# shayneobrien/generative-models

Measured on NVIDIA H100. Metric: train_step_images_per_sec, higher is better.
Workload: dtype bf16

## Files before the change

### generative-models_b200/gm_b200/csrc/engine.cu

```cuda
#include <cstdarg>
#include <cstdio>
#include <cstring>
#include <map>
#include <string>
#include <vector>

#include "gm_b200.h"
#include "gemm_wgmma.cuh"
#include "kernels.cuh"
#include "conv_ops.cuh"

using namespace gm;

typedef CUresult (*PFN_encodeTiled)(CUtensorMap*, CUtensorMapDataType, cuuint32_t, void*, const cuuint64_t*,
                                    const cuuint64_t*, const cuuint32_t*, const cuuint32_t*, CUtensorMapInterleave,
                                    CUtensorMapSwizzle, CUtensorMapL2promotion, CUtensorMapFloatOOBfill);

struct gm_ctx {
  int device = 0;
  int num_sms = 0;
  PFN_encodeTiled encode = nullptr;
  std::string err;
  long long launches = 0;
  float* scratch = nullptr;
// ... 22 lines not shown
    if (e__ != cudaSuccess)                                                                       \
      return fail(ctx, GM_ERR_CUDA, "%s failed: %s (%s:%d)", #expr, cudaGetErrorString(e__), __FILE__, __LINE__); \
  } while (0)

static inline int cdiv(int a, int b) { return (a + b - 1) / b; }
static inline int rup(int a, int b) { return cdiv(a, b) * b; }

static inline uint64_t splitmix64(uint64_t x) {
  x += 0x9E3779B97F4A7C15ull; x = (x ^ (x >> 30)) * 0xBF58476D1CE4E5B9ull; x = (x ^ (x >> 27)) * 0x94D049BB133111EBull;
  return x ^ (x >> 31);
}
static Sampler make_sampler(long long n, uint64_t seed, uint64_t round, uint64_t offset, const unsigned long long* step_ptr = nullptr) {
  Sampler sp;
  sp.n = n > 0 ? unsigned(n) : 0u;
  int bits = 2;
  while (bits < 32 && (1ull << bits) < (unsigned long long)(n > 0 ? n : 1)) ++bits;
  if (bits & 1) ++bits;
  sp.half_bits = unsigned(bits / 2);
  sp.seed_mix = splitmix64(seed);
  sp.key = sampler_key(sp.seed_mix, round);
  sp.offset = offset;
  sp.step_ptr = step_ptr;
  return sp;
}
static const Sampler kNoSampler = {0u, 1u, 0ull, 0ull, nullptr, 0ull};

static int make_tmap(gm_ctx* c, CUtensorMap* tm, const void* ptr, uint64_t inner, uint64_t outer, uint64_t ld,
                     uint32_t box_inner, uint32_t box_outer, CUtensorMapSwizzle swizzle = CU_TENSOR_MAP_SWIZZLE_128B) {
  if ((reinterpret_cast<uintptr_t>(ptr) & 15) || (ld * 2) % 16 != 0)
    return fail(c, GM_ERR_ARG, "tensor map: pointer/ld must be 16-byte aligned (ptr=%p ld=%llu)", ptr, (unsigned long long)ld);
  cuuint64_t dims[2] = {inner, outer};
  cuuint64_t strides[1] = {ld * 2};
  cuuint32_t box[2] = {box_inner, box_outer};
  cuuint32_t estr[2] = {1, 1};
  CUresult r = c->encode(tm, CU_TENSOR_MAP_DATA_TYPE_BFLOAT16, 2, const_cast<void*>(ptr), dims, strides, box, estr,
                         CU_TENSOR_MAP_INTERLEAVE_NONE, swizzle, CU_TENSOR_MAP_L2_PROMOTION_L2_256B,
                         CU_TENSOR_MAP_FLOAT_OOB_FILL_NONE);
  if (r != CUDA_SUCCESS) return fail(c, GM_ERR_CUDA, "cuTensorMapEncodeTiled failed with %d", int(r));
  return GM_OK;
}

enum PlanKind { PK_NT_208 = 0, PK_NT_64, PK_TN_256, PK_TN_64 };

struct GemmPlan {
  CUtensorMap tmA, tmB;
  CUtensorMap tmA2, tmB2;
  mutable CUtensorMap tmC;
  mutable int tmc_state;
  GemmParams p;
  int kind;
  int grid;
  double flops;
};

static bool g_pdl = true;
static bool g_tma_store = true;
struct ProfAll { const char* name; cudaEvent_t e0, e1; };
static bool g_prof_all = false;
static std::vector<ProfAll> g_prof_all_recs;
template <typename... KArgs, typename... Args>
static cudaError_t launch_pdl(const char* name, void (*kern)(KArgs...), dim3 grid, dim3 block, size_t smem, cudaStream_t s, Args&&... args) {
  struct Scope {
    cudaStream_t s; ProfAll r; bool on;
    Scope(const char* n, cudaStream_t s_) : s(s_), on(g_prof_all) {
      if (on) { r.name = n; cudaEventCreate(&r.e0); cudaEventCreate(&r.e1); cudaEventRecord(r.e0, s); }
    }
    ~Scope() { if (on) { cudaEventRecord(r.e1, s); g_prof_all_recs.push_back(r); } }
  } scope(name, s);
  const bool pdl = g_pdl && strcmp(name, "xhat_kernel") != 0;
  cudaLaunchConfig_t cfg;
  memset(&cfg, 0, sizeof cfg);
  cfg.gridDim = grid;
  cfg.blockDim = block;
  cfg.dynamicSmemBytes = smem;
  cfg.stream = s;
  cudaLaunchAttribute at[1];
  at[0].id = cudaLaunchAttributeProgrammaticStreamSerialization;
  at[0].val.programmaticStreamSerializationAllowed = 1;
  cfg.attrs = at;
  cfg.numAttrs = pdl ? 1 : 0;
  return cudaLaunchKernelEx(&cfg, kern, KArgs(args)...);
}

template <int BN, bool AMN, bool BMN, int ACT_T = -1, int AUX_T = -1, int BIAS_T = -1, int DOT_T = -1, bool SPLIT = false>
static cudaError_t launch_inst(const GemmPlan& pl, cudaStream_t s) {
  using Cfg = GemmCfg<BN, !AMN>;
  constexpr int CL = kGemmCluster<BN, AMN, BMN>;
  auto kern = gemm_wgmma_kernel<BN, AMN, BMN, ACT_T, AUX_T, BIAS_T, DOT_T, SPLIT>;
  cudaLaunchConfig_t cfg;
  memset(&cfg, 0, sizeof cfg);
  cfg.gridDim = dim3(pl.grid);
  cfg.blockDim = dim3(kGemmThreads);
  cfg.dynamicSmemBytes = Cfg::SMEM_BYTES;
  cfg.stream = s;
  cudaLaunchAttribute at[2];
  int na = 0;
  if (CL > 1) {
    at[na].id = cudaLaunchAttributeClusterDimension;
    at[na].val.clusterDim.x = CL;
    at[na].val.clusterDim.y = 1;
    at[na].val.clusterDim.z = 1;
    ++na;
  }
  static bool configured[64] = {};
  static int max_clusters[64] = {};
  int dev = 0;
  cudaGetDevice(&dev);
  const bool cached = dev >= 0 && dev < 64;
  int mc = cached ? max_clusters[dev] : 0;
  if (!cached || !configured[dev]) {
    cudaError_t e = cudaFuncSetAttribute(kern, cudaFuncAttributeMaxDynamicSharedMemorySize, Cfg::SMEM_BYTES);
    if (e != cudaSuccess) return e;
    if (CL > 1) {
      cfg.gridDim = dim3(CL);
      cfg.attrs = at;
      cfg.numAttrs = na;
      e = cudaOccupancyMaxActiveClusters(&mc, kern, &cfg);
      if (e != cudaSuccess) return e;
      if (mc < 1) return cudaErrorInvalidConfiguration;
    }
    if (cached) { max_clusters[dev] = mc; configured[dev] = true; }
  }
  if (CL > 1) {
    const GemmParams& q = pl.p;
    const int items = cdiv(q.m_tiles, CL) * q.n_tiles * q.splits;
    cfg.gridDim = dim3(CL * (items < mc ? items : mc));
  }
  if (g_pdl) {
    at[na].id = cudaLaunchAttributeProgrammaticStreamSerialization;
    at[na].val.programmaticStreamSerializationAllowed = 1;
    ++na;
  }
  cfg.attrs = at;
  cfg.numAttrs = na;
  GemmParams prm = pl.p;
  prm.tma_store = pl.tmc_state == 1 ? 1 : 0;
  prm.f32_vec = prm.epi == EPI_F32 && !(reinterpret_cast<uintptr_t>(prm.part) & 15) && prm.ldp % 4 == 0 && prm.part_stride % 4 == 0;
  return cudaLaunchKernelEx(&cfg, kern, pl.tmA, pl.tmB, pl.tmC, pl.tmA2, pl.tmB2, prm);
}

template <int BN, bool AMN, bool BMN>
static cudaError_t launch_split(const GemmPlan& pl, cudaStream_t s) {
  return launch_inst<BN, AMN, BMN, -1, -1, -1, -1, true>(pl, s);
}

static cudaError_t launch_nt208(const GemmPlan& pl, cudaStream_t s) {
  const GemmParams& p = pl.p;
  const bool bias = p.bias != nullptr, dot = p.dot_w != nullptr;
  const int aux = p.aux_mode;
  if (p.epi != EPI_BF16) return launch_inst<208, false, false>(pl, s);
  if (p.dot_sq && (bias || dot || aux != AUX_NONE || p.act != ACT_NONE)) return launch_inst<208, false, false>(pl, s);
  if (bias && !dot && aux == AUX_NONE && p.act == ACT_RELU) return launch_inst<208, false, false, ACT_RELU, AUX_NONE, 1, 0>(pl, s);
  if (bias && !dot && aux == AUX_NONE && p.act == ACT_SIGMOID) return launch_inst<208, false, false, ACT_SIGMOID, AUX_NONE, 1, 0>(pl, s);
  if (bias && dot && p.dot_mask == 1 && aux == AUX_NONE && p.act == ACT_RELU) return launch_inst<208, false, false, ACT_RELU, AUX_NONE, 1, 3>(pl, s);
  if (bias && dot && p.dot_mask == 3 && aux == AUX_NONE && p.act == ACT_RELU) return launch_inst<208, false, false, ACT_RELU, AUX_NONE, 1, 5>(pl, s);
  if (p.dot_mask) return launch_inst<208, false, false>(pl, s);
  if (bias && dot && aux == AUX_NONE && p.act == ACT_RELU) return launch_inst<208, false, false, ACT_RELU, AUX_NONE, 1, 1>(pl, s);
  if (!bias && !dot && aux == AUX_SIGMOID_GRAD && p.act == ACT_NONE) return launch_inst<208, false, false, ACT_NONE, AUX_SIGMOID_GRAD, 0, 0>(pl, s);
  if (!bias && !dot && aux == AUX_RELU_MASK && p.act == ACT_NONE) return launch_inst<208, false, false, ACT_NONE, AUX_RELU_MASK, 0, 0>(pl, s);
  if (!bias && !dot && aux == AUX_NONZERO_MASK && p.act == ACT_NONE) return launch_inst<208, false, false, ACT_NONE, AUX_NONZERO_MASK, 0, 0>(pl, s);
  if (bias && !dot && aux == AUX_L1 && p.act == ACT_NONE) return launch_inst<208, false, false, ACT_NONE, AUX_L1, 1, 0>(pl, s);
  if (bias && !dot && aux == AUX_VAE_OUT && p.act == ACT_SIGMOID) return launch_inst<208, false, false, ACT_SIGMOID, AUX_VAE_OUT, 1, 0>(pl, s);
  if (!bias && !dot && aux == AUX_NONE && p.act == ACT_NONE && p.dot_sq) return launch_inst<208, false, false, ACT_NONE, AUX_NONE, 0, 2>(pl, s);
  if (!bias && !dot && aux == AUX_NONE && p.act == ACT_NONE) return launch_inst<208, false, false, ACT_NONE, AUX_NONE, 0, 0>(pl, s);
  return launch_inst<208, false, false>(pl, s);
}

static int launch_plan(gm_ctx* c, const GemmPlan& pl, cudaStream_t s) {
  if (pl.tmc_state == 0) {
    const GemmParams& p = pl.p;
    const bool nt = pl.kind == PK_NT_208 || pl.kind == PK_NT_64;
    pl.tmc_state = 2;
    const bool plain = p.aux_mode == AUX_NONE && p.dot_w == nullptr && p.dot_sq == 0;
    if (g_tma_store && nt && plain && p.nparts == 1 && p.epi == EPI_BF16 && p.out != nullptr && !(reinterpret_cast<uintptr_t>(p.out) & 15) &&
        (p.ldo * 2) % 16 == 0 && p.out_cols > 0) {
      int rc = make_tmap(c, &pl.tmC, p.out, uint64_t(p.out_cols), uint64_t(p.M), uint64_t(p.ldo), kEpiCols, kEpiRows, CU_TENSOR_MAP_SWIZZLE_64B);
      if (rc) return rc;
      pl.tmc_state = 1;
    }
  }
  cudaError_t e;
  gm_ctx::ProfRec rec;
  ProfAll pa;
  if (g_prof_all) {
    static const char* kKind[4] = {"gemm_nt208", "gemm_nt64", "gemm_tn256", "gemm_tn64"};
    static std::map<int, std::string> names;
    const GemmParams& q = pl.p;
    const int key = pl.kind | (q.act << 4) | (q.aux_mode << 8) | ((q.dot_w != nullptr) << 12) | (q.dot_sq << 14) |
                    ((q.bias != nullptr) << 15) | ((q.epi == EPI_F32) << 16) | ((q.K >= 512) << 17) | ((q.nparts == 3) << 18) | (q.dot_mask << 19);
    auto it = names.find(key);
    if (it == names.end()) {
      char buf[128];
      snprintf(buf, sizeof buf, "%s[act%d aux%d%s%s%s%s%s K%s%s]", kKind[pl.kind], q.act, q.aux_mode, q.bias ? " bias" : "", q.dot_w ? " dot" : "",
               q.dot_mask == 3 ? " pre" : (q.dot_mask ? " mask" : ""), q.dot_sq ? " sq" : "", q.epi == EPI_F32 ? " f32" : "", q.K >= 512 ? "long" : "short", q.nparts == 3 ? " split" : "");
      it = names.emplace(key, buf).first;
    }
    pa.name = it->second.c_str();
    cudaEventCreate(&pa.e0); cudaEventCreate(&pa.e1);
    cudaEventRecord(pa.e0, s);
  }
  if (c->prof) {
    cudaEventCreate(&rec.e0);
    cudaEventCreate(&rec.e1);
    rec.kind = pl.kind;
    rec.flops = pl.flops;
    cudaEventRecord(rec.e0, s);
  }
  if (pl.p.nparts == 3) {
    switch (pl.kind) {
      case PK_NT_208: e = launch_split<208, false, false>(pl, s); break;
      case PK_NT_64: e = launch_split<64, false, false>(pl, s); break;
      case PK_TN_256: e = launch_split<256, true, true>(pl, s); break;
      default: e = launch_split<64, true, true>(pl, s); break;
    }
  } else
  switch (pl.kind) {
    case PK_NT_208: e = launch_nt208(pl, s); break;
    case PK_NT_64: e = launch_inst<64, false, false>(pl, s); break;
    case PK_TN_256: e = launch_inst<256, true, true>(pl, s); break;
    default: e = launch_inst<64, true, true>(pl, s); break;
  }
  c->launches++;
  if (c->prof) {
    cudaEventRecord(rec.e1, s);
    c->prof_recs.push_back(rec);
  }
  if (g_prof_all) { cudaEventRecord(pa.e1, s); g_prof_all_recs.push_back(pa); }
  if (e != cudaSuccess) return fail(c, GM_ERR_CUDA, "GEMM launch failed: %s", cudaGetErrorString(e));
  return GM_OK;
}

static int plan_gemm(gm_ctx* c, GemmPlan* pl, int mode, int M, int N, int K, const void* A, int lda, const void* B,
                     int ldb, int ncover, int max_splits) {
  memset(pl, 0, sizeof *pl);
  if (M <= 0 || N <= 0 || K <= 0) return fail(c, GM_ERR_ARG, "gemm: bad extents %d %d %d", M, N, K);
  int bn, boxn = 0;
  if (mode == 0) {
    if (ncover <= 64) { pl->kind = PK_NT_64; bn = 64; boxn = 64; }
    else { pl->kind = PK_NT_208; bn = 208; boxn = 208 / kGemmCluster<208, false, false>; }
    int rc = make_tmap(c, &pl->tmA, A, K, M, lda, BK, BM);
    if (rc) return rc;
    rc = make_tmap(c, &pl->tmB, B, K, N, ldb, BK, boxn);
    if (rc) return rc;
  } else {
    if (ncover <= 64) { pl->kind = PK_TN_64; bn = 64; }
    else { pl->kind = PK_TN_256; bn = 256; }
    int rc = make_tmap(c, &pl->tmA, A, M, K, lda, 64, BK);
    if (rc) return rc;
    rc = make_tmap(c, &pl->tmB, B, N, K, ldb, 64, BK);
    if (rc) return rc;
  }
  GemmParams& p = pl->p;
  pl->flops = 2.0 * M * N * K;
  p.M = M; p.N = N; p.K = K;
  p.m_tiles = cdiv(M, BM);
  p.n_tiles = cdiv(ncover, bn);
  p.kblocks = cdiv(K, BK);
  p.nparts = 1; p.kb_part = p.kblocks; p.lo_off = 0;
  pl->tmA2 = pl->tmA; pl->tmB2 = pl->tmB;
  if (c->plan_lo > 0) {
    const __nv_bfloat16* A2 = static_cast<const __nv_bfloat16*>(A) + c->plan_lo;
    const __nv_bfloat16* B2 = static_cast<const __nv_bfloat16*>(B) + c->plan_lo;
    int rc;
    if (mode == 0) {
      if ((rc = make_tmap(c, &pl->tmA2, A2, K, M, lda, BK, BM))) return rc;
      if ((rc = make_tmap(c, &pl->tmB2, B2, K, N, ldb, BK, boxn))) return rc;
    } else {
      if ((rc = make_tmap(c, &pl->tmA2, A2, M, K, lda, 64, BK))) return rc;
      if ((rc = make_tmap(c, &pl->tmB2, B2, N, K, ldb, 64, BK))) return rc;
    }
    p.nparts = 3; p.kblocks = 3 * p.kb_part; p.lo_off = c->plan_lo;
  }
  const int tiles = p.m_tiles * p.n_tiles;
  const int slots = c->num_sms;
  int splits = 1;
  if (max_splits > 1) {
    splits = slots / tiles;
    if (splits > max_splits) splits = max_splits;
    if (splits > p.kblocks) splits = p.kblocks;
    if (splits < 1) splits = 1;
  }
  p.kb_per_split = cdiv(p.kblocks, splits);
  p.splits = cdiv(p.kblocks, p.kb_per_split);
  const int total = tiles * p.splits;
  pl->grid = total < slots ? total : slots;
  return GM_OK;
}

__global__ void reduce_partials_kernel(const float* __restrict__ part, int nsplit, long long stride, long long rows, int cols,
                                       int ld, float* __restrict__ out) {
  griddep_sync();
  const long long k = blockIdx.x * (long long)blockDim.x + threadIdx.x;
  if (k >= rows * cols) return;
  const long long i = cols == ld ? k : (k / cols) * ld + k % cols;
  float t = 0.f;
  for (int s0 = 0; s0 < nsplit; s0 += 8) {
    float a[8];
#pragma unroll
    for (int u = 0; u < 8; ++u) a[u] = (s0 + u < nsplit) ? part[i + (long long)(s0 + u) * stride] : 0.f;
#pragma unroll
    for (int u = 0; u < 8; ++u) t += a[u];
  }
  out[i] = t;
}

extern "C" int gm_version(void) { return 100; }

extern "C" int gm_ctx_create(int device, gm_ctx** out) {
  if (!out) return GM_ERR_ARG;
  *out = nullptr;
  gm_ctx* c = new gm_ctx();
  c->device = device;
  *out = c;
  int n = 0;
  if (cudaGetDeviceCount(&n) != cudaSuccess || n <= 0)
    return fail(c, GM_ERR_CUDA, "no CUDA device visible: this library has no CPU fallback");
  CU_OK(c, cudaSetDevice(device));
  cudaDeviceProp prop;
  CU_OK(c, cudaGetDeviceProperties(&prop, device));
  if (prop.major != 9 || prop.minor != 0)
    return fail(c, GM_ERR_UNSUPPORTED, "device is sm_%d%d; this library is built for sm_90a (H100) only", prop.major, prop.minor);
  c->num_sms = prop.multiProcessorCount;
  void* fn = nullptr;
  cudaDriverEntryPointQueryResult q;
  CU_OK(c, cudaGetDriverEntryPoint("cuTensorMapEncodeTiled", &fn, cudaEnableDefault, &q));
  if (!fn || q != cudaDriverEntryPointSuccess) return fail(c, GM_ERR_CUDA, "cuTensorMapEncodeTiled not available");
  c->encode = reinterpret_cast<PFN_encodeTiled>(fn);
  const char* np = getenv("GM_NO_PDL");
  g_pdl = !(np && np[0] == '1');
  const char* nts = getenv("GM_NO_TMA_STORE");
  g_tma_store = !(nts && nts[0] == '1');
  return GM_OK;
}
extern "C" int gm_ctx_destroy(gm_ctx* c) {
  if (!c) return GM_OK;
  if (c->scratch) cudaFree(c->scratch);
  if (c->red) cudaFree(c->red);
  if (c->loss_zero) cudaFree(c->loss_zero);
  delete c;
  return GM_OK;
}
extern "C" const char* gm_last_error(const gm_ctx* c) { return c ? c->err.c_str() : "null ctx"; }
extern "C" int gm_ctx_num_sms(const gm_ctx* c) { return c ? c->num_sms : 0; }
extern "C" long long gm_launch_count(gm_ctx* c, int reset) {
  if (!c) return 0;
  const long long n = c->launches;
  if (reset) c->launches = 0;
  return n;
// ... 1219 lines not shown
```

### generative-models_b200/gm_b200/csrc/gemm_wgmma.cuh

```cuda
#pragma once
#include "ptx.cuh"

namespace gm {

constexpr int BM = 128;
constexpr int BK = 64;
constexpr int kMmaK = 16;
constexpr int kProducerThreads = 128;
constexpr int kConsumerWarps = 8;
constexpr int kGemmThreads = kProducerThreads + kConsumerWarps * 32;
constexpr int kProducerRegs = 40;
constexpr int kConsumerRegs = 232;
static_assert(kProducerThreads * kProducerRegs + kConsumerWarps * 32 * kConsumerRegs <= 65536, "register file");
constexpr int kSmemBudget = 227 * 1024;

enum : int { EPI_BF16 = 0, EPI_F32 = 1 };
enum : int { ACT_NONE = 0, ACT_RELU = 1, ACT_SIGMOID = 2, ACT_LRELU = 3 };
enum : int { AUX_NONE = 0, AUX_SIGMOID_GRAD = 1, AUX_RELU_MASK = 2, AUX_VAE_OUT = 3, AUX_L1 = 4, AUX_NONZERO_MASK = 5 };

struct GemmParams {
  int M, N, K;
  int m_tiles, n_tiles;
  int splits, kblocks, kb_per_split;
  int epi;
  __nv_bfloat16* out;
  int ldo;
  int out_cols;
  int pad_one;
  const float* bias;
  int act;
  const __nv_bfloat16* aux;
  int ld_aux;
  int aux_mode;
  const float* dot_w;
  int dot_sq;
  const float* row_scale;
  int row_split;
  int dot_mask;
  int tma_store;
  const float* row_vec;
  float* dot_out;
  int dot_ld;
  float* part;
  long long part_stride;
  int ldp;
  int transpose;
  int f32_vec;
  int nparts, kb_part;
  long long lo_off;
  float act_slope;
};

constexpr int kEpiRows = 16;
constexpr int kEpiStep = 64;
constexpr int kEpiCols = 32;
constexpr int kEpiScratchBytes = kEpiRows * kEpiStep * 4;
constexpr int kEpiPitch = 144;
constexpr int kEpiVecBlocks = 8;
constexpr int kEpiVecBytes = kEpiVecBlocks * kEpiCols * 4 * 2;
static_assert(kEpiRows * kEpiPitch <= kEpiScratchBytes && 2 * kEpiRows * kEpiCols * 2 <= kEpiScratchBytes, "staging");
__device__ __forceinline__ uint32_t frag_swz(int r) { return uint32_t(((r & 3) << 1) | ((r >> 2) & 1)); }

template <int BN_, bool STAGED_EPI = true>
struct GemmCfg {
  static constexpr int BN = BN_;
  static constexpr int A_BYTES = BM * BK * 2;
  static constexpr int B_BYTES = BN * BK * 2;
  static constexpr int STAGE_BYTES = A_BYTES + B_BYTES;
  static constexpr int EPI_BYTES = kConsumerWarps * (kEpiScratchBytes + (STAGED_EPI ? kEpiVecBytes : 0));
  static_assert(!STAGED_EPI || (BN + kEpiCols - 1) / kEpiCols <= kEpiVecBlocks, "bias/dot staging too small");
  static constexpr int FIXED_BYTES = 1024 + 512 + EPI_BYTES;
  static constexpr int STAGES_RAW = (kSmemBudget - FIXED_BYTES) / STAGE_BYTES;
  static constexpr int STAGES = STAGES_RAW > 8 ? 8 : STAGES_RAW;
  static constexpr int SMEM_BYTES = STAGES * STAGE_BYTES + FIXED_BYTES;
  static constexpr int BOXN = BN;
  static_assert(BN % 16 == 0 && BN <= 256, "wgmma N constraint (and 16-column epilogue chunks)");
  static_assert(STAGES >= 2, "need a pipeline");
  static_assert(BN < 208 || STAGES >= 4, "the 208- and 256-wide kernels need a 4-stage ring to hide TMA latency");
};

template <int BN, bool A_MN, bool B_MN>
constexpr int kGemmCluster = (BN == 208 && !A_MN && !B_MN) ? 2 : 1;

template <int BN, bool A_MN, bool B_MN, int ACT_T = -1, int AUX_T = -1, int BIAS_T = -1, int DOT_T = -1, bool SPLIT = false>
__global__ void __launch_bounds__(kGemmThreads, 1)
gemm_wgmma_kernel(const __grid_constant__ CUtensorMap tmA, const __grid_constant__ CUtensorMap tmB,
                  const __grid_constant__ CUtensorMap tmC, const __grid_constant__ CUtensorMap tmA2,
                  const __grid_constant__ CUtensorMap tmB2, const GemmParams p) {
  static_assert(!SPLIT || ACT_T < 0, "split operands: universal epilogue only");
  using Cfg = GemmCfg<BN, !A_MN>;
  constexpr int STAGES = Cfg::STAGES;
  constexpr int CL = kGemmCluster<BN, A_MN, B_MN>;
  static_assert(!B_MN || BN % 64 == 0, "MN-major B needs 64-wide atoms");
  static_assert(CL == 1 || (!B_MN && (BN / CL) % 8 == 0 && (Cfg::B_BYTES / CL) % 1024 == 0), "multicast B share");

  extern __shared__ uint8_t smem_raw[];
  const uint32_t smem_base = (smem_u32(smem_raw) + 1023u) & ~1023u;
  const uint32_t bar_base = smem_base + STAGES * Cfg::STAGE_BYTES;
  auto full_bar = [&](int s) { return bar_base + 8u * s; };
  auto empty_bar = [&](int s) { return bar_base + 8u * (STAGES + s); };
  const uint32_t epi_base = bar_base + 512u;

  const int warp = __shfl_sync(0xffffffffu, int(threadIdx.x >> 5), 0);
  const int lane = threadIdx.x & 31;

  griddep_launch();
  if (warp == 0 && lane == 0) {
    tma_prefetch_desc(&tmA);
    tma_prefetch_desc(&tmB);
    if constexpr (SPLIT) { tma_prefetch_desc(&tmA2); tma_prefetch_desc(&tmB2); }
    if (p.tma_store) tma_prefetch_desc(&tmC);
    for (int s = 0; s < STAGES; ++s) {
      mbar_init(full_bar(s), 1);
      mbar_init(empty_bar(s), CL * kConsumerWarps);
    }
    fence_mbar_init();
  }
  if constexpr (CL > 1) cluster_sync();
  else __syncthreads();
  griddep_wait();

  const int rank = CL > 1 ? int(cluster_ctarank()) : 0;
  const int tiles = (p.m_tiles + CL - 1) / CL * p.n_tiles;
  const int total = tiles * p.splits;
  const int first = blockIdx.x / CL, stride = gridDim.x / CL;

  if (warp < kProducerThreads / 32) {
    setmaxnreg_dec<kProducerRegs>();
    if (warp == 0) {
      int stage = 0;
      uint32_t phase = 0;
      const bool leader = elect_one();
      for (int item = first; item < total; item += stride) {
        const int split = item / tiles;
        const int rem = item - split * tiles;
        const int m0 = ((rem / p.n_tiles) * CL + rank) * BM;
        const int n0 = (rem % p.n_tiles) * BN;
        const int kb0 = split * p.kb_per_split;
        const int kb1 = min(kb0 + p.kb_per_split, p.kblocks);
        for (int kb = kb0; kb < kb1; ++kb) {
          mbar_wait(empty_bar(stage), phase ^ 1u);
          if (leader) {
            const uint32_t a_dst = smem_base + stage * Cfg::STAGE_BYTES;
            const uint32_t b_dst = a_dst + Cfg::A_BYTES;
            int kk = kb, opart = 0;
            if constexpr (SPLIT) { opart = kb / p.kb_part; kk = kb - opart * p.kb_part; }
            const CUtensorMap* const ta = (SPLIT && opart == 2) ? &tmA2 : &tmA;
            const CUtensorMap* const tb = (SPLIT && opart == 1) ? &tmB2 : &tmB;
            const int k0 = kk * BK;
            mbar_arrive_expect_tx(full_bar(stage), Cfg::STAGE_BYTES);
            if constexpr (!A_MN) {
              tma_load_2d(a_dst, ta, full_bar(stage), k0, m0);
            } else {
#pragma unroll
              for (int a = 0; a < BM / 64; ++a)
                tma_load_2d(a_dst + a * (BK * 128), ta, full_bar(stage), m0 + a * 64, k0);
            }
            if constexpr (CL > 1) {
              tma_load_2d_multicast(b_dst + rank * (Cfg::B_BYTES / CL), tb, full_bar(stage), k0, n0 + rank * (BN / CL), (1u << CL) - 1);
            } else if constexpr (!B_MN) {
              tma_load_2d(b_dst, tb, full_bar(stage), k0, n0);
            } else {
#pragma unroll
              for (int b = 0; b < BN / 64; ++b)
                tma_load_2d(b_dst + b * (BK * 128), tb, full_bar(stage), n0 + b * 64, k0);
            }
          }
          __syncwarp();
          if (++stage == STAGES) { stage = 0; phase ^= 1u; }
        }
      }
    }
  } else {
    setmaxnreg_inc<kConsumerRegs>();
    const int cw = warp - kProducerThreads / 32;
    const int wg = cw >> 2;
    const int er = lane & 15;
    const int par = lane >> 4;
    const uint32_t scratch_s = epi_base + uint32_t(cw) * kEpiScratchBytes;
    const uint32_t vec_s = epi_base + kConsumerWarps * kEpiScratchBytes + uint32_t(cw) * kEpiVecBytes;
    const int act = ACT_T >= 0 ? ACT_T : p.act;
    const int aux_mode = AUX_T >= 0 ? AUX_T : p.aux_mode;
    const bool has_bias = BIAS_T >= 0 ? (BIAS_T != 0) : (p.bias != nullptr);
    const bool has_dot = DOT_T >= 0 ? (DOT_T == 1 || DOT_T == 3 || DOT_T == 5) : (p.dot_w != nullptr);
    const bool store_pre = DOT_T >= 0 ? (DOT_T == 5) : (p.dot_mask == 3);
    const bool mask_all = DOT_T >= 0 ? (DOT_T == 3) : (p.dot_mask == 1);
    const bool has_sq = DOT_T >= 0 ? (DOT_T == 2) : (p.dot_sq != 0);
    constexpr bool kTmaStore = !A_MN && !SPLIT && AUX_T <= 0 && DOT_T <= 0 && !(BN == 208 && ACT_T < 0);
    const bool tma_st = kTmaStore && p.tma_store != 0;
    bool st_pending = false;
    auto stage_acquire = [&]() {
      if (st_pending) {
        if (er == 0) bulk_wait_read();
        __syncwarp();
        st_pending = false;
      }
    };
    constexpr uint32_t A_LBO = A_MN ? BK * 128 : 16, A_KADV = A_MN ? kMmaK * 128 : kMmaK * 2;
    constexpr uint32_t B_LBO = B_MN ? BK * 128 : 16, B_KADV = B_MN ? kMmaK * 128 : kMmaK * 2;
    constexpr uint32_t A_WG_OFF = A_MN ? BK * 128 : 64 * 128;
    constexpr uint32_t DESC_HI = (1024u >> 4) | (1u << 30);
    constexpr int kSteps = (BN + kEpiStep - 1) / kEpiStep;
    float acc[BN / 2];
    auto frag_to_scratch = [&](int s) {
#pragma unroll
      for (int t = 0; t < kSteps; ++t) {
        if (t == s) {
#pragma unroll
          for (int jj = 0; jj < kEpiStep / 8; ++jj) {
            const int j = t * (kEpiStep / 8) + jj;
            if (j < BN / 8) {
#pragma unroll
              for (int h = 0; h < 2; ++h) {
                const int r = (lane >> 2) + 8 * h, c = 8 * jj + 2 * (lane & 3);
                const uint32_t a = scratch_s + uint32_t(r) * (kEpiStep * 4) + ((uint32_t(c >> 2) ^ frag_swz(r)) << 4) + uint32_t(c & 3) * 4;
                asm volatile("st.shared.v2.f32 [%0], {%1, %2};" ::"r"(a), "f"(acc[4 * j + 2 * h]), "f"(acc[4 * j + 2 * h + 1]) : "memory");
              }
            }
          }
        }
      }
    };
    auto scratch_ld16 = [&](int c, uint32_t (&r)[16]) {
#pragma unroll
      for (int i = 0; i < 4; ++i) {
        const uint4 v = lds128(scratch_s + uint32_t(er) * (kEpiStep * 4) + ((uint32_t((c >> 2) + i) ^ frag_swz(er)) << 4));
        r[4 * i] = v.x; r[4 * i + 1] = v.y; r[4 * i + 2] = v.z; r[4 * i + 3] = v.w;
      }
    };
    auto release = [&](int s) {
      __syncwarp();
      if (lane == 0) {
        mbar_arrive(empty_bar(s));
        if constexpr (CL > 1) mbar_arrive_cluster(mapa_shared(empty_bar(s), uint32_t(rank ^ 1)));
      }
    };
    int stage = 0;
    uint32_t phase = 0;
#pragma unroll 1
    for (int item = first; item < total; item += stride) {
      const int split = item / tiles;
      const int rem = item - split * tiles;
      const int n_tile = rem % p.n_tiles;
      const int m0 = ((rem / p.n_tiles) * CL + rank) * BM;
      const int n0 = n_tile * BN;
      const int kb0 = split * p.kb_per_split;
      const int kb1 = min(kb0 + p.kb_per_split, p.kblocks);
      int prev = -1;
#pragma unroll 1
      for (int kb = kb0; kb < kb1; ++kb) {
        mbar_wait(full_bar(stage), phase);
        const uint32_t a_src = smem_base + stage * Cfg::STAGE_BYTES + wg * A_WG_OFF;
        const uint32_t b_src = smem_base + stage * Cfg::STAGE_BYTES + Cfg::A_BYTES;
        const uint32_t a_lo = ((a_src >> 4) & 0x3FFFu) | ((A_LBO >> 4) << 16);
        const uint32_t b_lo = ((b_src >> 4) & 0x3FFFu) | ((B_LBO >> 4) << 16);
        wgmma_pin(acc);
        wgmma_fence();
#pragma unroll
        for (int k = 0; k < BK / kMmaK; ++k) {
          const uint64_t da = (uint64_t(DESC_HI) << 32) | (a_lo + k * (A_KADV >> 4));
          const uint64_t db = (uint64_t(DESC_HI) << 32) | (b_lo + k * (B_KADV >> 4));
          const uint32_t sc = (kb > kb0 || k > 0) ? 1u : 0u;
          if constexpr (BN == 256) wgmma_bf16_n256<A_MN, B_MN>(acc, da, db, sc);
          else if constexpr (BN == 208) wgmma_bf16_n208<A_MN, B_MN>(acc, da, db, sc);
          else wgmma_bf16_n64<A_MN, B_MN>(acc, da, db, sc);
        }
        wgmma_commit();
        wgmma_wait<1>();
        wgmma_pin(acc);
        if (prev >= 0) release(prev);
        prev = stage;
        if (++stage == STAGES) { stage = 0; phase ^= 1u; }
      }
      wgmma_wait<0>();
      wgmma_pin(acc);
      if (prev >= 0) release(prev);
      const int wrow0 = m0 + wg * 64 + (cw & 3) * 16;
      const int row = wrow0 + er;
      const bool row_ok = row < p.M;
      constexpr bool kUniversal = ACT_T < 0;
      if (!A_MN && !(kUniversal && p.epi == EPI_F32)) {
        const int lr = lane >> 3, lc = lane & 7;
        constexpr int kBlocks = (BN + kEpiCols - 1) / kEpiCols;
        constexpr bool kAuxAsync = (AUX_T > 0) && (DOT_T == 0) && (BIAS_T == 0);
        const uint32_t auxt_s = vec_s;
        uint4 pre[kAuxAsync ? 1 : 4];
        auto aux_fetch = [&](int cs) {
          const int c = n0 + cs + lc * 8;
#pragma unroll
          for (int it = 0; it < 4; ++it) {
            const int rl = it * 4 + lr;
            const int r = wrow0 + rl;
            const bool ok = r < p.M && c < p.out_cols && cs + lc * 8 < BN;
            if constexpr (kAuxAsync) {
              const __nv_bfloat16* src = ok ? p.aux + size_t(r) * p.ld_aux + c : p.aux;
              cp_async16_zfill(auxt_s + rl * 128 + ((lc ^ (rl & 7)) << 4), src, ok ? 16u : 0u);
            } else {
              pre[it] = make_uint4(0, 0, 0, 0);
              if (ok) pre[it] = __ldg(reinterpret_cast<const uint4*>(p.aux + size_t(r) * p.ld_aux + c));
            }
          }
          if constexpr (kAuxAsync) cp_async_commit();
        };
        if (has_bias || has_dot) {
#pragma unroll
          for (int pass = 0; pass < kEpiVecBlocks / 4; ++pass) {
            const int blk = pass * 4 + (lane >> 3), c4 = (lane & 7) * 4;
            const int c = n0 + blk * kEpiCols + c4;
            uint4 bz = make_uint4(0, 0, 0, 0), wz = bz;
            if (blk < kBlocks && c < p.N) {
              if (has_bias) {
                bz = __ldg(reinterpret_cast<const uint4*>(p.bias + c));
                if (act == ACT_SIGMOID) {
                  bz.x = __float_as_uint(0.5f * __uint_as_float(bz.x)); bz.y = __float_as_uint(0.5f * __uint_as_float(bz.y));
                  bz.z = __float_as_uint(0.5f * __uint_as_float(bz.z)); bz.w = __float_as_uint(0.5f * __uint_as_float(bz.w));
                }
              }
              if (has_dot) wz = __ldg(reinterpret_cast<const uint4*>(p.dot_w + c));
            }
            if (has_bias) sts128(vec_s + (blk * kEpiCols + c4) * 4, bz);
            if (has_dot) sts128(vec_s + kEpiVecBytes / 2 + (blk * kEpiCols + c4) * 4, wz);
          }
          __syncwarp();
        }
        if (aux_mode != AUX_NONE) {
          aux_fetch(0);
          const int nitem = item + stride;
          if (nitem < total) {
            const int nrem = nitem - (nitem / tiles) * tiles;
            const int nm0 = ((nrem / p.n_tiles) * CL + rank) * BM + wg * 64 + (cw & 3) * 16;
            const int nn0 = (nrem % p.n_tiles) * BN;
            for (int t = lane; t < kEpiRows * 4; t += 32) {
              const int r = nm0 + (t >> 2), c = nn0 + (t & 3) * 64;
              if (r < p.M && c < p.out_cols)
                asm volatile("prefetch.global.L2 [%0];" ::"l"(p.aux + size_t(r) * p.ld_aux + c));
            }
          }
        }
        float dot = 0.f;
        float l1_scale = 0.f;
        if (aux_mode == AUX_L1) l1_scale = __ldg(p.row_scale + (row < p.row_split ? 0 : 1));
        if (aux_mode == AUX_SIGMOID_GRAD || aux_mode == AUX_RELU_MASK || aux_mode == AUX_NONZERO_MASK) l1_scale = (p.row_vec != nullptr && row_ok) ? __ldg(p.row_vec + row) : 1.f;
#pragma unroll 1
        for (int s = 0; s < kSteps; ++s) {
          const int cs = s * kEpiStep;
          if (n0 + cs >= p.out_cols) break;
          const int bi = 2 * s + par;
          const int cb = bi * kEpiCols;
          const int col0 = n0 + cb;
          const int nch = (cb >= BN || col0 >= p.out_cols) ? 0 : (BN - cb) >= kEpiCols ? 2 : (BN - cb) / 16;
          const bool last_step = (cs + kEpiStep >= BN) || (n0 + cs + kEpiStep >= p.out_cols);
          const bool step_tma = tma_st && BN - cs >= kEpiStep && wrow0 < p.M;
          stage_acquire();
          frag_to_scratch(s);
          __syncwarp();
// ... 228 lines not shown
```

### generative-models_b200/gm_b200/csrc/ptx.cuh

```cuda
#pragma once
#include <cstdint>
#include <cuda.h>
#include <cuda_bf16.h>
#include <cuda_runtime.h>

namespace gm {

#ifndef GM_WATCHDOG_CYCLES
#define GM_WATCHDOG_CYCLES (4000000000LL)
#endif

__device__ __forceinline__ uint32_t smem_u32(const void* p) {
  return static_cast<uint32_t>(__cvta_generic_to_shared(p));
}

__device__ __forceinline__ bool elect_one() {
  uint32_t pred;
  asm volatile(
      "{\n"
      ".reg .pred p;\n"
      "elect.sync _|p, 0xffffffff;\n"
      "selp.u32 %0, 1, 0, p;\n"
      "}\n"
      : "=r"(pred));
  return pred != 0;
}

__device__ __forceinline__ void mbar_init(uint32_t bar, uint32_t count) {
  asm volatile("mbarrier.init.shared::cta.b64 [%0], %1;" ::"r"(bar), "r"(count) : "memory");
}
__device__ __forceinline__ void fence_mbar_init() {
  asm volatile("fence.mbarrier_init.release.cluster;" ::: "memory");
}
__device__ __forceinline__ void mbar_arrive_expect_tx(uint32_t bar, uint32_t bytes) {
  asm volatile("mbarrier.arrive.expect_tx.shared::cta.b64 _, [%0], %1;" ::"r"(bar), "r"(bytes) : "memory");
}
__device__ __forceinline__ void mbar_arrive(uint32_t bar) {
  asm volatile("mbarrier.arrive.shared::cta.b64 _, [%0];" ::"r"(bar) : "memory");
}
__device__ __forceinline__ bool mbar_try_wait(uint32_t bar, uint32_t parity) {
  uint32_t ok;
  asm volatile(
      "{\n"
      ".reg .pred p;\n"
      "mbarrier.try_wait.parity.shared::cta.b64 p, [%1], %2;\n"
      "selp.u32 %0, 1, 0, p;\n"
      "}\n"
      : "=r"(ok)
      : "r"(bar), "r"(parity)
      : "memory");
  return ok != 0;
}
__device__ __forceinline__ void mbar_wait(uint32_t bar, uint32_t parity) {
  if (mbar_try_wait(bar, parity)) return;
  const long long t0 = clock64();
  while (!mbar_try_wait(bar, parity)) {
    if (clock64() - t0 > GM_WATCHDOG_CYCLES) __trap();
  }
}

__device__ __forceinline__ uint32_t cluster_ctarank() {
  uint32_t r;
  asm("mov.u32 %0, %%cluster_ctarank;" : "=r"(r));
  return r;
}
__device__ __forceinline__ void cluster_sync() {
  asm volatile("barrier.cluster.arrive.release.aligned;\nbarrier.cluster.wait.acquire.aligned;" ::: "memory");
}
__device__ __forceinline__ uint32_t mapa_shared(uint32_t addr, uint32_t rank) {
  uint32_t r;
  asm("mapa.shared::cluster.u32 %0, %1, %2;" : "=r"(r) : "r"(addr), "r"(rank));
  return r;
}
__device__ __forceinline__ void mbar_arrive_cluster(uint32_t cluster_bar) {
  asm volatile("mbarrier.arrive.shared::cluster.b64 _, [%0];" ::"r"(cluster_bar) : "memory");
}

__device__ __forceinline__ void tma_prefetch_desc(const void* tmap) {
  asm volatile("prefetch.tensormap [%0];" ::"l"(reinterpret_cast<uint64_t>(tmap)) : "memory");
}
__device__ __forceinline__ void tma_load_2d(uint32_t smem_dst, const void* tmap, uint32_t bar, int c0, int c1) {
  asm volatile(
      "cp.async.bulk.tensor.2d.shared::cluster.global.mbarrier::complete_tx::bytes [%0], [%1, {%3, %4}], [%2];"
      ::"r"(smem_dst), "l"(reinterpret_cast<uint64_t>(tmap)), "r"(bar), "r"(c0), "r"(c1)
      : "memory");
}
__device__ __forceinline__ void tma_load_2d_multicast(uint32_t smem_dst, const void* tmap, uint32_t bar, int c0, int c1, uint16_t cta_mask) {
  asm volatile(
      "cp.async.bulk.tensor.2d.shared::cluster.global.mbarrier::complete_tx::bytes.multicast::cluster [%0], [%1, {%3, %4}], [%2], %5;"
      ::"r"(smem_dst), "l"(reinterpret_cast<uint64_t>(tmap)), "r"(bar), "r"(c0), "r"(c1), "h"(cta_mask)
      : "memory");
}

__device__ __forceinline__ void wgmma_fence() { asm volatile("wgmma.fence.sync.aligned;" ::: "memory"); }
__device__ __forceinline__ void wgmma_commit() { asm volatile("wgmma.commit_group.sync.aligned;" ::: "memory"); }
template <int N>
__device__ __forceinline__ void wgmma_wait() { asm volatile("wgmma.wait_group.sync.aligned %0;" ::"n"(N) : "memory"); }
template <int R>
__device__ __forceinline__ void wgmma_pin(float (&d)[R]) {
#pragma unroll
  for (int i = 0; i < R; ++i) asm volatile("" : "+f"(d[i])::"memory");
}

template <int TA, int TB>
__device__ __forceinline__ void wgmma_bf16_n64(float (&d)[32], uint64_t da, uint64_t db, uint32_t scale_d) {
  asm volatile(
      "{\n"
      ".reg .pred p;\n"
      "setp.ne.b32 p, %34, 0;\n"
      "wgmma.mma_async.sync.aligned.m64n64k16.f32.bf16.bf16 {%0,%1,%2,%3,%4,%5,%6,%7,%8,%9,%10,%11,%12,%13,%14,%15,%16,%17,%18,%19,%20,%21,%22,%23,%24,%25,%26,%27,%28,%29,%30,%31}, %32, %33, p, 1, 1, %35, %36;\n"
      "}\n"
      : "+f"(d[0]), "+f"(d[1]), "+f"(d[2]), "+f"(d[3]), "+f"(d[4]), "+f"(d[5]), "+f"(d[6]), "+f"(d[7]), "+f"(d[8]), "+f"(d[9]), "+f"(d[10]), "+f"(d[11]), "+f"(d[12]), "+f"(d[13]), "+f"(d[14]), "+f"(d[15]), "+f"(d[16]), "+f"(d[17]), "+f"(d[18]), "+f"(d[19]), "+f"(d[20]), "+f"(d[21]), "+f"(d[22]), "+f"(d[23]), "+f"(d[24]), "+f"(d[25]), "+f"(d[26]), "+f"(d[27]), "+f"(d[28]), "+f"(d[29]), "+f"(d[30]), "+f"(d[31])
      : "l"(da), "l"(db), "r"(scale_d), "n"(TA), "n"(TB));
}

template <int TA, int TB>
__device__ __forceinline__ void wgmma_bf16_n208(float (&d)[104], uint64_t da, uint64_t db, uint32_t scale_d) {
  asm volatile(
      "{\n"
      ".reg .pred p;\n"
      "setp.ne.b32 p, %106, 0;\n"
      "wgmma.mma_async.sync.aligned.m64n208k16.f32.bf16.bf16 {%0,%1,%2,%3,%4,%5,%6,%7,%8,%9,%10,%11,%12,%13,%14,%15,%16,%17,%18,%19,%20,%21,%22,%23,%24,%25,%26,%27,%28,%29,%30,%31,%32,%33,%34,%35,%36,%37,%38,%39,%40,%41,%42,%43,%44,%45,%46,%47,%48,%49,%50,%51,%52,%53,%54,%55,%56,%57,%58,%59,%60,%61,%62,%63,%64,%65,%66,%67,%68,%69,%70,%71,%72,%73,%74,%75,%76,%77,%78,%79,%80,%81,%82,%83,%84,%85,%86,%87,%88,%89,%90,%91,%92,%93,%94,%95,%96,%97,%98,%99,%100,%101,%102,%103}, %104, %105, p, 1, 1, %107, %108;\n"
      "}\n"
      : "+f"(d[0]), "+f"(d[1]), "+f"(d[2]), "+f"(d[3]), "+f"(d[4]), "+f"(d[5]), "+f"(d[6]), "+f"(d[7]), "+f"(d[8]), "+f"(d[9]), "+f"(d[10]), "+f"(d[11]), "+f"(d[12]), "+f"(d[13]), "+f"(d[14]), "+f"(d[15]), "+f"(d[16]), "+f"(d[17]), "+f"(d[18]), "+f"(d[19]), "+f"(d[20]), "+f"(d[21]), "+f"(d[22]), "+f"(d[23]), "+f"(d[24]), "+f"(d[25]), "+f"(d[26]), "+f"(d[27]), "+f"(d[28]), "+f"(d[29]), "+f"(d[30]), "+f"(d[31]), "+f"(d[32]), "+f"(d[33]), "+f"(d[34]), "+f"(d[35]), "+f"(d[36]), "+f"(d[37]), "+f"(d[38]), "+f"(d[39]), "+f"(d[40]), "+f"(d[41]), "+f"(d[42]), "+f"(d[43]), "+f"(d[44]), "+f"(d[45]), "+f"(d[46]), "+f"(d[47]), "+f"(d[48]), "+f"(d[49]), "+f"(d[50]), "+f"(d[51]), "+f"(d[52]), "+f"(d[53]), "+f"(d[54]), "+f"(d[55]), "+f"(d[56]), "+f"(d[57]), "+f"(d[58]), "+f"(d[59]), "+f"(d[60]), "+f"(d[61]), "+f"(d[62]), "+f"(d[63]), "+f"(d[64]), "+f"(d[65]), "+f"(d[66]), "+f"(d[67]), "+f"(d[68]), "+f"(d[69]), "+f"(d[70]), "+f"(d[71]), "+f"(d[72]), "+f"(d[73]), "+f"(d[74]), "+f"(d[75]), "+f"(d[76]), "+f"(d[77]), "+f"(d[78]), "+f"(d[79]), "+f"(d[80]), "+f"(d[81]), "+f"(d[82]), "+f"(d[83]), "+f"(d[84]), "+f"(d[85]), "+f"(d[86]), "+f"(d[87]), "+f"(d[88]), "+f"(d[89]), "+f"(d[90]), "+f"(d[91]), "+f"(d[92]), "+f"(d[93]), "+f"(d[94]), "+f"(d[95]), "+f"(d[96]), "+f"(d[97]), "+f"(d[98]), "+f"(d[99]), "+f"(d[100]), "+f"(d[101]), "+f"(d[102]), "+f"(d[103])
      : "l"(da), "l"(db), "r"(scale_d), "n"(TA), "n"(TB));
}

template <int TA, int TB>
__device__ __forceinline__ void wgmma_bf16_n256(float (&d)[128], uint64_t da, uint64_t db, uint32_t scale_d) {
  asm volatile(
      "{\n"
      ".reg .pred p;\n"
      "setp.ne.b32 p, %130, 0;\n"
      "wgmma.mma_async.sync.aligned.m64n256k16.f32.bf16.bf16 {%0,%1,%2,%3,%4,%5,%6,%7,%8,%9,%10,%11,%12,%13,%14,%15,%16,%17,%18,%19,%20,%21,%22,%23,%24,%25,%26,%27,%28,%29,%30,%31,%32,%33,%34,%35,%36,%37,%38,%39,%40,%41,%42,%43,%44,%45,%46,%47,%48,%49,%50,%51,%52,%53,%54,%55,%56,%57,%58,%59,%60,%61,%62,%63,%64,%65,%66,%67,%68,%69,%70,%71,%72,%73,%74,%75,%76,%77,%78,%79,%80,%81,%82,%83,%84,%85,%86,%87,%88,%89,%90,%91,%92,%93,%94,%95,%96,%97,%98,%99,%100,%101,%102,%103,%104,%105,%106,%107,%108,%109,%110,%111,%112,%113,%114,%115,%116,%117,%118,%119,%120,%121,%122,%123,%124,%125,%126,%127}, %128, %129, p, 1, 1, %131, %132;\n"
      "}\n"
      : "+f"(d[0]), "+f"(d[1]), "+f"(d[2]), "+f"(d[3]), "+f"(d[4]), "+f"(d[5]), "+f"(d[6]), "+f"(d[7]), "+f"(d[8]), "+f"(d[9]), "+f"(d[10]), "+f"(d[11]), "+f"(d[12]), "+f"(d[13]), "+f"(d[14]), "+f"(d[15]), "+f"(d[16]), "+f"(d[17]), "+f"(d[18]), "+f"(d[19]), "+f"(d[20]), "+f"(d[21]), "+f"(d[22]), "+f"(d[23]), "+f"(d[24]), "+f"(d[25]), "+f"(d[26]), "+f"(d[27]), "+f"(d[28]), "+f"(d[29]), "+f"(d[30]), "+f"(d[31]), "+f"(d[32]), "+f"(d[33]), "+f"(d[34]), "+f"(d[35]), "+f"(d[36]), "+f"(d[37]), "+f"(d[38]), "+f"(d[39]), "+f"(d[40]), "+f"(d[41]), "+f"(d[42]), "+f"(d[43]), "+f"(d[44]), "+f"(d[45]), "+f"(d[46]), "+f"(d[47]), "+f"(d[48]), "+f"(d[49]), "+f"(d[50]), "+f"(d[51]), "+f"(d[52]), "+f"(d[53]), "+f"(d[54]), "+f"(d[55]), "+f"(d[56]), "+f"(d[57]), "+f"(d[58]), "+f"(d[59]), "+f"(d[60]), "+f"(d[61]), "+f"(d[62]), "+f"(d[63]), "+f"(d[64]), "+f"(d[65]), "+f"(d[66]), "+f"(d[67]), "+f"(d[68]), "+f"(d[69]), "+f"(d[70]), "+f"(d[71]), "+f"(d[72]), "+f"(d[73]), "+f"(d[74]), "+f"(d[75]), "+f"(d[76]), "+f"(d[77]), "+f"(d[78]), "+f"(d[79]), "+f"(d[80]), "+f"(d[81]), "+f"(d[82]), "+f"(d[83]), "+f"(d[84]), "+f"(d[85]), "+f"(d[86]), "+f"(d[87]), "+f"(d[88]), "+f"(d[89]), "+f"(d[90]), "+f"(d[91]), "+f"(d[92]), "+f"(d[93]), "+f"(d[94]), "+f"(d[95]), "+f"(d[96]), "+f"(d[97]), "+f"(d[98]), "+f"(d[99]), "+f"(d[100]), "+f"(d[101]), "+f"(d[102]), "+f"(d[103]), "+f"(d[104]), "+f"(d[105]), "+f"(d[106]), "+f"(d[107]), "+f"(d[108]), "+f"(d[109]), "+f"(d[110]), "+f"(d[111]), "+f"(d[112]), "+f"(d[113]), "+f"(d[114]), "+f"(d[115]), "+f"(d[116]), "+f"(d[117]), "+f"(d[118]), "+f"(d[119]), "+f"(d[120]), "+f"(d[121]), "+f"(d[122]), "+f"(d[123]), "+f"(d[124]), "+f"(d[125]), "+f"(d[126]), "+f"(d[127])
      : "l"(da), "l"(db), "r"(scale_d), "n"(TA), "n"(TB));
}

template <int N>
__device__ __forceinline__ void setmaxnreg_dec() { asm volatile("setmaxnreg.dec.sync.aligned.u32 %0;" ::"n"(N)); }
template <int N>
__device__ __forceinline__ void setmaxnreg_inc() { asm volatile("setmaxnreg.inc.sync.aligned.u32 %0;" ::"n"(N)); }

__device__ __forceinline__ void sts128(uint32_t addr, uint4 v) {
  asm volatile("st.shared.v4.b32 [%0], {%1,%2,%3,%4};" ::"r"(addr), "r"(v.x), "r"(v.y), "r"(v.z), "r"(v.w) : "memory");
}
__device__ __forceinline__ uint4 lds128(uint32_t addr) {
  uint4 v;
  asm volatile("ld.shared.v4.b32 {%0,%1,%2,%3}, [%4];" : "=r"(v.x), "=r"(v.y), "=r"(v.z), "=r"(v.w) : "r"(addr) : "memory");
  return v;
}

__device__ __forceinline__ uint64_t make_smem_desc(uint32_t smem_addr, uint32_t lbo_bytes, uint32_t sbo_bytes) {
  uint64_t d = 0;
  d |= static_cast<uint64_t>((smem_addr >> 4) & 0x3FFFu);
  d |= static_cast<uint64_t>((lbo_bytes >> 4) & 0x3FFFu) << 16;
  d |= static_cast<uint64_t>((sbo_bytes >> 4) & 0x3FFFu) << 32;
// ... 65 lines not shown
```

Baseline: 41.58 million.

## Add ping-pong consumer warpgroup schedule for short-K 208-wide bias GEMMs

Adds a ping-pong mode to the 128x208 K-major WGMMA kernel. Each consumer warpgroup now owns a whole 64-row half-tile, and the two warpgroups take turns issuing MMAs through named barriers, so one group's epilogue overlaps the other's main loop. The producer loads A as 64-row half tiles into a smaller stage with a 5-stage ring. The mode is enabled only for bias+ReLU/sigmoid epilogues with at most 7 K-blocks, where epilogue time is comparable to MMA time. In exchange, the named-barrier turn-taking adds serialization and handshake complexity, and the A tensor map box is now halved for every NT-208 GEMM.

```diff
diff --git a/generative-models_b200/gm_b200/csrc/engine.cu b/generative-models_b200/gm_b200/csrc/engine.cu
--- a/generative-models_b200/gm_b200/csrc/engine.cu
+++ b/generative-models_b200/gm_b200/csrc/engine.cu
@@ -128,11 +128,12 @@
   return cudaLaunchKernelEx(&cfg, kern, KArgs(args)...);
 }
 
-template <int BN, bool AMN, bool BMN, int ACT_T = -1, int AUX_T = -1, int BIAS_T = -1, int DOT_T = -1, bool SPLIT = false>
+template <int BN, bool AMN, bool BMN, int ACT_T = -1, int AUX_T = -1, int BIAS_T = -1, int DOT_T = -1, bool SPLIT = false,
+          bool PP = false>
 static cudaError_t launch_inst(const GemmPlan& pl, cudaStream_t s) {
-  using Cfg = GemmCfg<BN, !AMN>;
+  using Cfg = GemmCfg<BN, !AMN, PP>;
   constexpr int CL = kGemmCluster<BN, AMN, BMN>;
-  auto kern = gemm_wgmma_kernel<BN, AMN, BMN, ACT_T, AUX_T, BIAS_T, DOT_T, SPLIT>;
+  auto kern = gemm_wgmma_kernel<BN, AMN, BMN, ACT_T, AUX_T, BIAS_T, DOT_T, SPLIT, PP>;
   cudaLaunchConfig_t cfg;
   memset(&cfg, 0, sizeof cfg);
   cfg.gridDim = dim3(pl.grid);
@@ -190,14 +191,21 @@
   return launch_inst<BN, AMN, BMN, -1, -1, -1, -1, true>(pl, s);
 }
 
+constexpr int kPingPongMaxKblocks = 7;
+
 static cudaError_t launch_nt208(const GemmPlan& pl, cudaStream_t s) {
   const GemmParams& p = pl.p;
   const bool bias = p.bias != nullptr, dot = p.dot_w != nullptr;
   const int aux = p.aux_mode;
   if (p.epi != EPI_BF16) return launch_inst<208, false, false>(pl, s);
   if (p.dot_sq && (bias || dot || aux != AUX_NONE || p.act != ACT_NONE)) return launch_inst<208, false, false>(pl, s);
-  if (bias && !dot && aux == AUX_NONE && p.act == ACT_RELU) return launch_inst<208, false, false, ACT_RELU, AUX_NONE, 1, 0>(pl, s);
-  if (bias && !dot && aux == AUX_NONE && p.act == ACT_SIGMOID) return launch_inst<208, false, false, ACT_SIGMOID, AUX_NONE, 1, 0>(pl, s);
+  const bool pp = p.kblocks <= kPingPongMaxKblocks;
+  if (bias && !dot && aux == AUX_NONE && p.act == ACT_RELU)
+    return pp ? launch_inst<208, false, false, ACT_RELU, AUX_NONE, 1, 0, false, true>(pl, s)
+              : launch_inst<208, false, false, ACT_RELU, AUX_NONE, 1, 0>(pl, s);
+  if (bias && !dot && aux == AUX_NONE && p.act == ACT_SIGMOID)
+    return pp ? launch_inst<208, false, false, ACT_SIGMOID, AUX_NONE, 1, 0, false, true>(pl, s)
+              : launch_inst<208, false, false, ACT_SIGMOID, AUX_NONE, 1, 0>(pl, s);
   if (bias && dot && p.dot_mask == 1 && aux == AUX_NONE && p.act == ACT_RELU) return launch_inst<208, false, false, ACT_RELU, AUX_NONE, 1, 3>(pl, s);
   if (bias && dot && p.dot_mask == 3 && aux == AUX_NONE && p.act == ACT_RELU) return launch_inst<208, false, false, ACT_RELU, AUX_NONE, 1, 5>(pl, s);
   if (p.dot_mask) return launch_inst<208, false, false>(pl, s);
@@ -280,11 +288,13 @@
                      int ldb, int ncover, int max_splits) {
   memset(pl, 0, sizeof *pl);
   if (M <= 0 || N <= 0 || K <= 0) return fail(c, GM_ERR_ARG, "gemm: bad extents %d %d %d", M, N, K);
-  int bn, boxn = 0;
+  int bn, boxn = 0, boxm = BM;
   if (mode == 0) {
     if (ncover <= 64) { pl->kind = PK_NT_64; bn = 64; boxn = 64; }
-    else { pl->kind = PK_NT_208; bn = 208; boxn = 208 / kGemmCluster<208, false, false>; }
-    int rc = make_tmap(c, &pl->tmA, A, K, M, lda, BK, BM);
+    else {
+      pl->kind = PK_NT_208; bn = 208; boxn = 208 / kGemmCluster<208, false, false>; boxm = kGemmABoxRows<208, false>;
+    }
+    int rc = make_tmap(c, &pl->tmA, A, K, M, lda, BK, boxm);
     if (rc) return rc;
     rc = make_tmap(c, &pl->tmB, B, K, N, ldb, BK, boxn);
     if (rc) return rc;
@@ -309,7 +319,7 @@
     const __nv_bfloat16* B2 = static_cast<const __nv_bfloat16*>(B) + c->plan_lo;
     int rc;
     if (mode == 0) {
-      if ((rc = make_tmap(c, &pl->tmA2, A2, K, M, lda, BK, BM))) return rc;
+      if ((rc = make_tmap(c, &pl->tmA2, A2, K, M, lda, BK, boxm))) return rc;
       if ((rc = make_tmap(c, &pl->tmB2, B2, K, N, ldb, BK, boxn))) return rc;
     } else {
       if ((rc = make_tmap(c, &pl->tmA2, A2, M, K, lda, 64, BK))) return rc;
diff --git a/generative-models_b200/gm_b200/csrc/gemm_wgmma.cuh b/generative-models_b200/gm_b200/csrc/gemm_wgmma.cuh
--- a/generative-models_b200/gm_b200/csrc/gemm_wgmma.cuh
+++ b/generative-models_b200/gm_b200/csrc/gemm_wgmma.cuh
@@ -9,6 +9,8 @@
 constexpr int kProducerThreads = 128;
 constexpr int kConsumerWarps = 8;
 constexpr int kGemmThreads = kProducerThreads + kConsumerWarps * 32;
+constexpr int kBarWg0Issued = 1;
+constexpr int kBarWg1Issued = 2;
 constexpr int kProducerRegs = 40;
 constexpr int kConsumerRegs = 232;
 static_assert(kProducerThreads * kProducerRegs + kConsumerWarps * 32 * kConsumerRegs <= 65536, "register file");
@@ -61,10 +63,16 @@
 static_assert(kEpiRows * kEpiPitch <= kEpiScratchBytes && 2 * kEpiRows * kEpiCols * 2 <= kEpiScratchBytes, "staging");
 __device__ __forceinline__ uint32_t frag_swz(int r) { return uint32_t(((r & 3) << 1) | ((r >> 2) & 1)); }
 
-template <int BN_, bool STAGED_EPI = true>
+template <int BN, bool A_MN>
+constexpr int kGemmABoxRows = (BN == 208 && !A_MN) ? BM / 2 : BM;
+
+template <int BN_, bool STAGED_EPI = true, bool PINGPONG_ = false>
 struct GemmCfg {
   static constexpr int BN = BN_;
-  static constexpr int A_BYTES = BM * BK * 2;
+  static constexpr bool PINGPONG = PINGPONG_;
+  static_assert(!PINGPONG || (STAGED_EPI && BN == 208), "ping-pong: 128 x 208 K-major kernel only");
+  static constexpr int A_ROWS = PINGPONG ? BM / 2 : BM;
+  static constexpr int A_BYTES = A_ROWS * BK * 2;
   static constexpr int B_BYTES = BN * BK * 2;
   static constexpr int STAGE_BYTES = A_BYTES + B_BYTES;
   static constexpr int EPI_BYTES = kConsumerWarps * (kEpiScratchBytes + (STAGED_EPI ? kEpiVecBytes : 0));
@@ -77,20 +85,25 @@
   static_assert(BN % 16 == 0 && BN <= 256, "wgmma N constraint (and 16-column epilogue chunks)");
   static_assert(STAGES >= 2, "need a pipeline");
   static_assert(BN < 208 || STAGES >= 4, "the 208- and 256-wide kernels need a 4-stage ring to hide TMA latency");
+  static_assert(!PINGPONG || (STAGES == 5 && SMEM_BYTES <= kSmemBudget), "ping-pong ring");
 };
 
 template <int BN, bool A_MN, bool B_MN>
 constexpr int kGemmCluster = (BN == 208 && !A_MN && !B_MN) ? 2 : 1;
 
-template <int BN, bool A_MN, bool B_MN, int ACT_T = -1, int AUX_T = -1, int BIAS_T = -1, int DOT_T = -1, bool SPLIT = false>
+template <int BN, bool A_MN, bool B_MN, int ACT_T = -1, int AUX_T = -1, int BIAS_T = -1, int DOT_T = -1, bool SPLIT = false,
+          bool PINGPONG = false>
 __global__ void __launch_bounds__(kGemmThreads, 1)
 gemm_wgmma_kernel(const __grid_constant__ CUtensorMap tmA, const __grid_constant__ CUtensorMap tmB,
                   const __grid_constant__ CUtensorMap tmC, const __grid_constant__ CUtensorMap tmA2,
                   const __grid_constant__ CUtensorMap tmB2, const GemmParams p) {
   static_assert(!SPLIT || ACT_T < 0, "split operands: universal epilogue only");
-  using Cfg = GemmCfg<BN, !A_MN>;
+  using Cfg = GemmCfg<BN, !A_MN, PINGPONG>;
   constexpr int STAGES = Cfg::STAGES;
   constexpr int CL = kGemmCluster<BN, A_MN, B_MN>;
+  constexpr bool PP = PINGPONG;
+  constexpr int A_BOX = kGemmABoxRows<BN, A_MN>;
+  static_assert(Cfg::A_ROWS % A_BOX == 0, "A tile in whole boxes");
   static_assert(!B_MN || BN % 64 == 0, "MN-major B needs 64-wide atoms");
   static_assert(CL == 1 || (!B_MN && (BN / CL) % 8 == 0 && (Cfg::B_BYTES / CL) % 1024 == 0), "multicast B share");
 
@@ -112,7 +125,7 @@
     if (p.tma_store) tma_prefetch_desc(&tmC);
     for (int s = 0; s < STAGES; ++s) {
       mbar_init(full_bar(s), 1);
-      mbar_init(empty_bar(s), CL * kConsumerWarps);
+      mbar_init(empty_bar(s), CL * (PP ? kConsumerWarps / 2 : kConsumerWarps));
     }
     fence_mbar_init();
   }
@@ -124,12 +137,17 @@
   const int tiles = (p.m_tiles + CL - 1) / CL * p.n_tiles;
   const int total = tiles * p.splits;
   const int first = blockIdx.x / CL, stride = gridDim.x / CL;
+  auto halves_of = [&](int rem) -> int {
+    if constexpr (PP) return (rem / p.n_tiles) * CL * BM + Cfg::A_ROWS < p.M ? 2 : 1;
+    else return 1;
+  };
+  auto stage_of = [](uint32_t it) { return int(it % STAGES); };
+  auto phase_of = [](uint32_t it) { return (it / STAGES) & 1u; };
 
   if (warp < kProducerThreads / 32) {
     setmaxnreg_dec<kProducerRegs>();
     if (warp == 0) {
-      int stage = 0;
-      uint32_t phase = 0;
+      uint32_t it = 0;
       const bool leader = elect_one();
       for (int item = first; item < total; item += stride) {
         const int split = item / tiles;
@@ -138,8 +156,11 @@
         const int n0 = (rem % p.n_tiles) * BN;
         const int kb0 = split * p.kb_per_split;
         const int kb1 = min(kb0 + p.kb_per_split, p.kblocks);
-        for (int kb = kb0; kb < kb1; ++kb) {
-          mbar_wait(empty_bar(stage), phase ^ 1u);
+        const int nh = halves_of(rem);
+        for (int h = 0; h < nh; ++h)
+        for (int kb = kb0; kb < kb1; ++kb, ++it) {
+          const int stage = stage_of(it);
+          mbar_wait(empty_bar(stage), phase_of(it) ^ 1u);
           if (leader) {
             const uint32_t a_dst = smem_base + stage * Cfg::STAGE_BYTES;
             const uint32_t b_dst = a_dst + Cfg::A_BYTES;
@@ -150,7 +171,9 @@
             const int k0 = kk * BK;
             mbar_arrive_expect_tx(full_bar(stage), Cfg::STAGE_BYTES);
             if constexpr (!A_MN) {
-              tma_load_2d(a_dst, ta, full_bar(stage), k0, m0);
+#pragma unroll
+              for (int a = 0; a < Cfg::A_ROWS / A_BOX; ++a)
+                tma_load_2d(a_dst + a * (A_BOX * BK * 2), ta, full_bar(stage), k0, m0 + h * Cfg::A_ROWS + a * A_BOX);
             } else {
 #pragma unroll
               for (int a = 0; a < BM / 64; ++a)
@@ -167,7 +190,6 @@
             }
           }
           __syncwarp();
-          if (++stage == STAGES) { stage = 0; phase ^= 1u; }
         }
       }
     }
@@ -237,6 +259,7 @@
     };
     int stage = 0;
     uint32_t phase = 0;
+    uint32_t it = 0;
 #pragma unroll 1
     for (int item = first; item < total; item += stride) {
       const int split = item / tiles;
@@ -246,11 +269,26 @@
       const int n0 = n_tile * BN;
       const int kb0 = split * p.kb_per_split;
       const int kb1 = min(kb0 + p.kb_per_split, p.kblocks);
+      const int nh = halves_of(rem);
+      if constexpr (PP) {
+        if (wg == 1 || it != 0) named_bar_sync(wg == 1 ? kBarWg0Issued : kBarWg1Issued, kConsumerWarps * 32);
+        if (wg == 1 && nh == 1) {
+          it += uint32_t(kb1 - kb0);
+          if (item + stride < total) named_bar_arrive(kBarWg1Issued, kConsumerWarps * 32);
+          continue;
+        }
+      }
       int prev = -1;
+      if constexpr (PP) {
+        const uint32_t it0 = it + (wg == 1 ? uint32_t(kb1 - kb0) : 0u);
+        stage = stage_of(it0);
+        phase = phase_of(it0);
+        it += uint32_t(nh * (kb1 - kb0));
+      }
 #pragma unroll 1
       for (int kb = kb0; kb < kb1; ++kb) {
         mbar_wait(full_bar(stage), phase);
-        const uint32_t a_src = smem_base + stage * Cfg::STAGE_BYTES + wg * A_WG_OFF;
+        const uint32_t a_src = smem_base + stage * Cfg::STAGE_BYTES + (PP ? 0u : wg * A_WG_OFF);
         const uint32_t b_src = smem_base + stage * Cfg::STAGE_BYTES + Cfg::A_BYTES;
         const uint32_t a_lo = ((a_src >> 4) & 0x3FFFu) | ((A_LBO >> 4) << 16);
         const uint32_t b_lo = ((b_src >> 4) & 0x3FFFu) | ((B_LBO >> 4) << 16);
@@ -271,6 +309,9 @@
         if (prev >= 0) release(prev);
         prev = stage;
         if (++stage == STAGES) { stage = 0; phase ^= 1u; }
+      }
+      if constexpr (PP) {
+        if (wg == 0 || item + stride < total) named_bar_arrive(wg == 0 ? kBarWg0Issued : kBarWg1Issued, kConsumerWarps * 32);
       }
       wgmma_wait<0>();
       wgmma_pin(acc);
diff --git a/generative-models_b200/gm_b200/csrc/ptx.cuh b/generative-models_b200/gm_b200/csrc/ptx.cuh
--- a/generative-models_b200/gm_b200/csrc/ptx.cuh
+++ b/generative-models_b200/gm_b200/csrc/ptx.cuh
@@ -74,6 +74,13 @@
 }
 __device__ __forceinline__ void mbar_arrive_cluster(uint32_t cluster_bar) {
   asm volatile("mbarrier.arrive.shared::cluster.b64 _, [%0];" ::"r"(cluster_bar) : "memory");
+}
+
+__device__ __forceinline__ void named_bar_sync(int id, int threads) {
+  asm volatile("bar.sync %0, %1;" ::"r"(id), "r"(threads) : "memory");
+}
+__device__ __forceinline__ void named_bar_arrive(int id, int threads) {
+  asm volatile("bar.arrive %0, %1;" ::"r"(id), "r"(threads) : "memory");
 }
 
 __device__ __forceinline__ void tma_prefetch_desc(const void* tmap) {
```

Measured after the change: 42.90 million (median of 6 runs). 1.03x the previous value.
